# Alxaline/BraTS21

Measured on AMD Instinct MI355X. Metric: train patches/sec (4x128^3, width-48), higher is better.
Workload: dtype bf16; 1 GPU; equiunet width=48, batch=2/GPU of 4x128^3 synthetic patches, fwd + deep-supervision Dice + bwd + ranger (BASELINE.json configs[1]); global_batch=2, parallelism=dp1

## Files before the change

### brats21_amd/csrc/conv_wgrad.hip

```cpp
#include <stdlib.h>
#include "twin_begin.hpp"
#include "common.hpp"

typedef __attribute__((ext_vector_type(4))) short s16x4;

struct WgradParams {
  const void* x1; const void* x2; int c1, c2, p1, p2;
  const void* dy; int dyp;
  float* ws;
  int N, D, H, W, cin, cout;
  int tz, ty, tx, ntiles, nsplit;
  int nlane;
  int ntaps, dil;
  int seglen, nsegz;
};

constexpr int WG_TZ = 4, WG_TY = 4, WG_TX = 16, WG_VOX = 256;

template <typename T, int DIL, int COF, int CIF, int KS = 3>
struct WgGeom {
  static constexpr bool BF = std::is_same<T, bf16_t>::value;
  static constexpr int ESZ = sizeof(T);
  static constexpr int EPL = 16 / ESZ;
  static constexpr int R = KS == 3 ? DIL : 0;
// ... 543 lines not shown
      const int yoff = ybase + (32 * s) * G::SY;
#pragma unroll
      for (int m = 0; m < COF; ++m) a[s & 1][m] = tr_pair(ldy + yoff + m * 32, ldy + yoff + 16 * G::SY + m * 32);
    };
    auto read_b = [&](auto u_) {
      constexpr int u = u_;
      constexpr int s = u / G::PPW, jj = u % G::PPW;
      const int xoff = xbase + (((s >> 1) * G::HY + 2 * (s & 1)) * G::HX) * G::SX + poff[jj];
      b[u % (PD + 1)] = tr_pair(ldx + xoff, ldx + xoff + G::HX * G::SX);
    };
    constexpr int NU = 8 * G::PPW;
    static_for<0, G::XI>([&](auto i_) { issue_x(L, i_); });
    static_for<0, G::YI>([&](auto i_) { issue_y(L, i_); });
    __builtin_amdgcn_sched_barrier(0);
    read_a(std::integral_constant<int, 0>{});
    static_for<0, PD>([&](auto u_) { read_b(u_); });
    static_for<0, NU>([&](auto u_) {
      constexpr int u = u_;
      constexpr int s = u / G::PPW, jj = u % G::PPW;
      if constexpr (u + PD < NU) read_b(std::integral_constant<int, u + PD>{});
      if constexpr (jj == 0 && s + 1 < 8) read_a(std::integral_constant<int, s + 1>{});
      __builtin_amdgcn_sched_barrier(0);
#pragma unroll
      for (int m = 0; m < COF; ++m)
        acc[jj][m] = MFMA16_16x16x32(a[s & 1][m], b[u % (PD + 1)], acc[jj][m]);
      __builtin_amdgcn_sched_barrier(0);
    });
  }

#ifdef BRATS_WGRAD_STAMPS
  WG_STAMP(4);
  if (lane == 0 && blockIdx.y == 0 && blockIdx.z == 0) {
    long long* st = (long long*)(p.ws + (size_t)gridDim.x * 27 * p.cout * p.cin) + ((size_t)blockIdx.x * 8 + wave) * 5;
    for (int i = 0; i < 5; ++i) st[i] = tacc[i];
  }
#endif
#pragma unroll
  for (int jj = 0; jj < G::PPW; ++jj) {
    const int pid = wave + 8 * jj;
    if (pid < G::PAIRS) {
      const int t = pid / CIF, nn = pid % CIF;
      float* base = p.ws + ((size_t)split * 27 + t) * p.cout * p.cin;
      const int ci = ci0 + nn * 16 + v;
      if (CIF > 1 || ci < p.cin) {
#pragma unroll
        for (int m = 0; m < COF; ++m)
#pragma unroll
          for (int r = 0; r < 4; ++r) base[(size_t)(co0 + m * 16 + 4 * q + r) * p.cin + ci] = acc[jj][m][r];
      }
    }
  }
}

template <int COF, int CIF> struct Wg3f {
  static constexpr int HZ = WG_TZ + 2, HY = WG_TY + 2, HX = WG_TX + 2, HVOX = HZ * HY * HX;
  static constexpr int CO = 16 * COF, CI = 16 * CIF;
  static constexpr int SX = CI, SY = CO;
  static constexpr int XPPV = CI / 8, YPPV = CO / 8;
  static constexpr int XPIECES = HVOX * XPPV, YPIECES = WG_VOX * YPPV;
  static constexpr int XI = (XPIECES + 511) / 512, YI = YPIECES / 512;
  static constexpr int XB = XI * 512 * 16, YB = YI * 512 * 16;
  static constexpr int LDS_X = HVOX * SX;
  static constexpr int LDS = XB + YB + LDS_X + WG_VOX * SY;
  static constexpr int PAIRS = 27 * CIF, PPW = (PAIRS + 7) / 8;
  static_assert(YPIECES % 512 == 0, "");
};

template <int STRIDE> DEVI i32x8 tr8_frag(const char* base, int o0, int o1) {
  typedef __attribute__((ext_vector_type(2))) int v2i;
  typedef __attribute__((address_space(3))) v2i* lp;
  const v2i a0 = __builtin_amdgcn_ds_read_tr8_b64_v2i32((lp)(base + o0));
  const v2i a1 = __builtin_amdgcn_ds_read_tr8_b64_v2i32((lp)(base + o0 + 8 * STRIDE));
  const v2i a2 = __builtin_amdgcn_ds_read_tr8_b64_v2i32((lp)(base + o1));
  const v2i a3 = __builtin_amdgcn_ds_read_tr8_b64_v2i32((lp)(base + o1 + 8 * STRIDE));
  return i32x8{a0[0], a0[1], a1[0], a1[1], a2[0], a2[1], a3[0], a3[1]};
}

struct WgradF8Params { WgradParams w; const float* amax_x1; const float* amax_x2; const float* amax_dy; };

template <int COF, int CIF>
__global__ __launch_bounds__(512, 1) void conv_wgrad_alltaps_f8_kernel(const WgradF8Params pp) {
  typedef bf16_t T;
  using G = Wg3f<COF, CIF>;
  const WgradParams& p = pp.w;
  extern __shared__ __attribute__((aligned(16))) char lds[];
  char* ldx = lds + G::XB + G::YB;
  char* ldy = ldx + G::LDS_X;
  const int tid = threadIdx.x, lane = tid & 63;
  const int wave = __builtin_amdgcn_readfirstlane(tid >> 6);
  const int kq = lane >> 4, L = lane & 15;
  const int lane8 = blockIdx.x % p.nlane, gsub = blockIdx.x / p.nlane, g8 = gridDim.x / p.nlane;
  const int split = blockIdx.x;
  const int tpx = (p.ntiles + p.nlane - 1) / p.nlane;
  const int tile_end = min(p.ntiles, (lane8 + 1) * tpx);
  const int co0 = blockIdx.y * G::CO, ci0 = blockIdx.z * G::CI;
  const T* xsrc;
  int xpitch;
  if (ci0 < p.c1) { xsrc = (const T*)p.x1 + ci0; xpitch = p.p1; }
  else { xsrc = (const T*)p.x2 + (ci0 - p.c1); xpitch = p.p2; }
  const int xpb = xpitch * 2, ypb = p.dyp * 2;
  float ax = *pp.amax_x1;
  if (pp.amax_x2) ax = fmaxf(ax, *pp.amax_x2);
  const float xs = f8_scale_from_amax(ax), ys = f8_scale_from_amax(*pp.amax_dy);

  int xoffs[G::XI], xcode[G::XI];
#pragma unroll
// ... 273 lines not shown
  return t;
}
static WgradParams wgrad_params(const WgradArgs& a, float* ws, const WgradTileGrid& t, int nlane, int nsplit, int ntaps, int dil) {
  WgradParams p{};
  p.x1 = a.x1; p.x2 = a.x2; p.c1 = a.c1; p.c2 = a.c2; p.p1 = a.p1; p.p2 = a.p2;
  p.dy = a.dy; p.dyp = a.dyp; p.ws = ws;
  p.N = a.N; p.D = a.D; p.H = a.H; p.W = a.W; p.cin = a.cin(); p.cout = a.cout;
  p.tz = t.tz; p.ty = t.ty; p.tx = t.tx; p.ntiles = t.ntiles;
  p.nlane = nlane; p.nsplit = nsplit; p.ntaps = ntaps; p.dil = dil;
  return p;
}

static int wgrad_nlane(int ntiles) {
  int nl = 8;
  while (nl > 1 && ntiles / nl < 16) nl >>= 1;
  return nl;
}
static int wgrad_split_g8(int ntiles, int nlane, int groups, int cot, int cit) {
  int g8 = ceil_div(512, groups * nlane * cot * cit);
  const int cap = ceil_div(ntiles, nlane);
  if (g8 > cap) g8 = cap;
  return g8 < 1 ? 1 : g8;
}
static bool wgrad_blocks_g8(int ntiles, int blocks, int* nlane, int* g8) {
  *nlane = wgrad_nlane(ntiles);
  *g8 = ceil_div(device_cus(), *nlane * blocks);
  if (*g8 < 1) *g8 = 1;
  return ntiles >= 4 * *nlane * *g8;
}
static void wgrad_tiles(int dtype, int c1, int c2, int cout, int* cof, int* cif) {
  const int co16 = ceil_div(cout, 16);
  *cof = co16 % 3 == 0 ? 3 : (co16 % 2 == 0 ? 2 : 1);
  if (dtype == BRATS_F32) { *cif = 1; return; }
  const int a = ceil_div(c1, 16), b = c2 > 0 ? ceil_div(c2, 16) : 0;
  auto ok = [&](int f) { return a % f == 0 && (b == 0 || b % f == 0); };
  *cif = ok(3) ? 3 : (ok(2) ? 2 : 1);
}

int g_wgrad_alltaps_mode = -1;
extern "C" int BRATS_API(brats_conv3d_set_wgrad_alltaps)(int mode) {
  const int old = g_wgrad_alltaps_mode;
  g_wgrad_alltaps_mode = mode < 0 ? -1 : (mode ? 1 : 0);
  return old;
}
static int wgrad_alltaps_mode() {
  static int env_mode = -1;
  if (env_mode < 0) {
    const char* e = getenv("BRATS_WGRAD_ALLTAPS");
    env_mode = e ? atoi(e) : 1;
  }
  return g_wgrad_alltaps_mode >= 0 ? g_wgrad_alltaps_mode : env_mode;
}

enum WgradForm {
  WG_TAP_PLANE, WG_SHIFTED_TAP,
  WG_ALLTAPS2_33, WG_ALLTAPS2_42, WG_ALLTAPS2_31,
  WG_ALLTAPS_1, WG_ALLTAPS_1_4,
  WG_F8_33, WG_F8_42
};
struct WgradPlan {
  WgradForm form;
  int cof, cif;
  int cot, cit;
  int nlane, g8, nsplit;
  int ntaps, groups;
  bool clear;
  WgradTileGrid tiles;
  size_t per;
  size_t slab_bytes() const { return nsplit * per * sizeof(float); }
};

static WgradPlan wgrad_plan(int dtype, bool shifted, int ksize, int dil, const WgradArgs& a) {
  WgradPlan pl;
  const int c1 = a.c1, c2 = a.c2, cin = a.cin(), cout = a.cout;
  pl.tiles = wgrad_tile_grid(a);
  pl.ntaps = ksize == 3 ? 27 : 1;
  pl.per = (size_t)pl.ntaps * cout * cin;
  const bool narrow = c2 == 0 && c1 <= 16;
  auto blocks_of = [&](int co, int ci) { return cout % co == 0 && (narrow || (c1 % ci == 0 && c2 % ci == 0)); };
  if (!shifted && wgrad_alltaps_mode() && dtype == BRATS_BF16 && dil == 1 && (blocks_of(48, 48) || blocks_of(64, 32))) {
    const bool wide = !blocks_of(48, 48);
    pl.cof = wide ? 4 : 3; pl.cif = narrow ? 1 : (wide ? 2 : 3);
    pl.cot = cout / (16 * pl.cof); pl.cit = narrow ? 1 : cin / (16 * pl.cif);
    if (wgrad_blocks_g8(pl.tiles.ntiles, pl.cot * pl.cit, &pl.nlane, &pl.g8)) {
      pl.form = wide ? (narrow ? WG_ALLTAPS_1_4 : WG_ALLTAPS2_42) : narrow ? (c1 % 8 == 0 ? WG_ALLTAPS2_31 : WG_ALLTAPS_1) : WG_ALLTAPS2_33;
      pl.groups = 1;
      pl.clear = false;
      pl.nsplit = pl.nlane * pl.g8;
      return pl;
    }
  }
  pl.form = shifted ? WG_SHIFTED_TAP : WG_TAP_PLANE;
  wgrad_tiles(dtype, c1, c2, cout, &pl.cof, &pl.cif);
  pl.cot = ceil_div(cout, 16 * pl.cof);
  pl.cit = ceil_div(c1, 16 * pl.cif) + (c2 > 0 ? ceil_div(c2, 16 * pl.cif) : 0);
  pl.groups = shifted ? pl.ntaps : 3;
  pl.nlane = wgrad_nlane(pl.tiles.ntiles);
  pl.g8 = wgrad_split_g8(pl.tiles.ntiles, pl.nlane, pl.groups, pl.cot, pl.cit);
  pl.nsplit = pl.nlane * pl.g8;
  pl.clear = cin % 16 || cout % 16;
  return pl;
}
static size_t wgrad_slab_room(int dtype, bool shifted, int ksize, const WgradArgs& a) {
  const size_t d1 = wgrad_plan(dtype, shifted, ksize, 1, a).slab_bytes();
  const size_t d2 = shifted ? 0 : wgrad_plan(dtype, shifted, ksize, 2, a).slab_bytes();
  return d1 > d2 ? d1 : d2;
}

template <typename T, int DIL, int COF, int CIF, int KS = 3>
static int wgrad_launch(const WgradParams& p, dim3 grid, hipStream_t st) {
  using G = WgGeom<T, DIL, COF, CIF, KS>;
  auto kern = conv_wgrad_kernel<T, DIL, COF, CIF, KS>;
  static std::atomic<uint64_t> attr_done{0};
  BRATS_ENSURE_LDS_ATTR(kern, G::LDS, attr_done);
  hipLaunchKernelGGL(kern, grid, dim3(256), G::LDS, st, p);
  BRATS_CHECK_LAUNCH();
  return 0;
}

template <typename T, int DIL, int KS = 3>
static int wgrad_dispatch(const WgradParams& p, int cof, int cif, dim3 grid, hipStream_t st) {
#define WG_CASE(A, B) if (cof == A && cif == B) return wgrad_launch<T, DIL, A, B, KS>(p, grid, st);
  WG_CASE(3, 1) WG_CASE(2, 1) WG_CASE(1, 1)
  if constexpr (std::is_same<T, bf16_t>::value) {
    WG_CASE(3, 3) WG_CASE(3, 2) WG_CASE(2, 3) WG_CASE(2, 2) WG_CASE(1, 3) WG_CASE(1, 2)
  }
#undef WG_CASE
  BRATS_FAIL(BRATS_E_UNSUPPORTED, "wgrad: unsupported tile %dx%d", cof, cif);
}

template <auto KERN, int LDS>
static int wgrad_alltaps_launch(const WgradParams& p, dim3 grid, hipStream_t st) {
  static std::atomic<uint64_t> attr_done{0};
  BRATS_ENSURE_LDS_ATTR(KERN, LDS, attr_done);
  hipLaunchKernelGGL(KERN, grid, dim3(512), LDS, st, p);
  BRATS_CHECK_LAUNCH();
  return 0;
}

static int wgrad_run(const WgradPlan& pl, int dtype, int dil, const WgradArgs& a, float* ws, size_t room, hipStream_t st) {
  const char* who = pl.form == WG_SHIFTED_TAP ? "wgrad_shift" : "wgrad";
  if (a.c2 > 0 && a.c1 % (16 * pl.cif)) BRATS_FAIL(BRATS_E_UNSUPPORTED, "wgrad: c1=%d must be a multiple of the ci tile %d", a.c1, 16 * pl.cif);
  if (pl.slab_bytes() > room) BRATS_FAIL(BRATS_E_ARG, "%s: the plan's %zu bytes of slabs exceed the workspace size %zu", who, pl.slab_bytes(), room);
  const WgradParams p = wgrad_params(a, ws, pl.tiles, pl.nlane, pl.nsplit, pl.ntaps, dil);
  if (pl.clear) {
    hipError_t e = hipMemsetAsync(ws, 0, pl.slab_bytes(), st);
    if (e != hipSuccess) BRATS_FAIL(BRATS_E_HIP, "%s: memset: %s", who, hipGetErrorString(e));
  }
  const dim3 grid(pl.groups * pl.nsplit, pl.cot, pl.cit);
  const bool bf = dtype == BRATS_BF16;
  switch (pl.form) {
    case WG_TAP_PLANE:
      if (bf) return dil == 1 ? wgrad_dispatch<bf16_t, 1>(p, pl.cof, pl.cif, grid, st) : wgrad_dispatch<bf16_t, 2>(p, pl.cof, pl.cif, grid, st);
      return dil == 1 ? wgrad_dispatch<float, 1>(p, pl.cof, pl.cif, grid, st) : wgrad_dispatch<float, 2>(p, pl.cof, pl.cif, grid, st);
    case WG_SHIFTED_TAP:
      return bf ? wgrad_dispatch<bf16_t, 1, 1>(p, pl.cof, pl.cif, grid, st) : wgrad_dispatch<float, 1, 1>(p, pl.cof, pl.cif, grid, st);
    case WG_ALLTAPS2_33: return wgrad_alltaps_launch<conv_wgrad_alltaps2_kernel<3, 3>, Wg3b<3, 3>::LDS>(p, grid, st);
    case WG_ALLTAPS2_42: return wgrad_alltaps_launch<conv_wgrad_alltaps2_kernel<4, 2>, Wg3b<4, 2>::LDS>(p, grid, st);
    case WG_ALLTAPS2_31: return wgrad_alltaps_launch<conv_wgrad_alltaps2_kernel<3, 1>, Wg3b<3, 1>::LDS>(p, grid, st);
    case WG_ALLTAPS_1: return wgrad_alltaps_launch<conv_wgrad_alltaps_kernel<1>, Wg3<1>::LDS>(p, grid, st);
    case WG_ALLTAPS_1_4: return wgrad_alltaps_launch<conv_wgrad_alltaps_kernel<1, 4>, Wg3<1, 4>::LDS>(p, grid, st);
    default: BRATS_FAIL(BRATS_E_UNSUPPORTED, "wgrad: form %d is not a 16-bit / f32 kernel", (int)pl.form);
  }
}

template <int V>
__global__ void __launch_bounds__(256) x3_split_kernel(const float* __restrict__ src, int pitch, bf16_t* __restrict__ hi,
                                                       bf16_t* __restrict__ lo, size_t voxels, int C, const float* __restrict__ amax) {
  const float sc = amax ? x3_scale_from_amax(*amax) : 1.f;
  const int cv = C / 8;
  const size_t total = voxels * cv;
  const size_t stride = (size_t)gridDim.x * 256;
  auto load = [&](size_t i, u32x4& a, u32x4& b) {
    const float* p = src + (i / cv) * pitch + (i % cv) * 8;
    a = __builtin_nontemporal_load((const u32x4*)p);
    b = __builtin_nontemporal_load((const u32x4*)(p + 4));
  };
  auto emit = [&](size_t i, const u32x4& a, const u32x4& b) {
    const uint32_t w[8] = {a[0], a[1], a[2], a[3], b[0], b[1], b[2], b[3]};
    uint32_t h[4], l[4];
#pragma unroll
    for (int e = 0; e < 4; ++e) {
      const float x0 = __uint_as_float(w[2 * e]) * sc, x1 = __uint_as_float(w[2 * e + 1]) * sc;
      x3_split2(x0, x1, h[e], l[e]);
    }
    const size_t o = (i / cv) * C + (i % cv) * 8;
    __builtin_nontemporal_store(u32x4{h[0], h[1], h[2], h[3]}, (u32x4*)(hi + o));
    __builtin_nontemporal_store(u32x4{l[0], l[1], l[2], l[3]}, (u32x4*)(lo + o));
  };
  size_t i = (size_t)blockIdx.x * 256 + threadIdx.x;
  for (; i + stride < total; i += 2 * stride) {
    u32x4 a0, b0, a1, b1;
    load(i, a0, b0);
    load(i + stride, a1, b1);
    emit(i, a0, b0);
    emit(i + stride, a1, b1);
  }
  if (i < total) {
    u32x4 a0, b0;
    load(i, a0, b0);
    emit(i, a0, b0);
  }
}
static size_t x3_align(size_t b) { return (b + 255) / 256 * 256; }
// ... 9 lines not shown
  X3Carve(size_t room16, const WgradArgs& a) {
    const int c[3] = {a.c1, a.c2, a.cout};
    size_t b = x3_align(3 * room16);
    for (int i = 0; i < 6; ++i) {
      off[i] = b;
      b += c[i / 2] > 0 ? x3_align(a.vox() * c[i / 2] * 2) : 0;
    }
    off[6] = b;
  }
  size_t bytes() const { return off[6]; }
  bf16_t* at(float* ws, int i) const { return (bf16_t*)((char*)ws + off[i]); }
};

static int wgrad_x3(const WgradPlan& pl, int dil, const WgradArgs& a, const float* amax_dy, float* ws, float* dw, size_t room16,
                          hipStream_t st) {
  const X3Carve cv(room16, a);
  bf16_t *h1 = cv.at(ws, 0), *l1 = cv.at(ws, 1), *h2 = cv.at(ws, 2), *l2 = cv.at(ws, 3), *hy = cv.at(ws, 4), *ly = cv.at(ws, 5);
  x3_split_launch((const float*)a.x1, a.p1, h1, l1, a.vox(), a.c1, nullptr, st);
  if (a.c2 > 0) x3_split_launch((const float*)a.x2, a.p2, h2, l2, a.vox(), a.c2, nullptr, st);
  x3_split_launch((const float*)a.dy, a.dyp, hy, ly, a.vox(), a.cout, amax_dy, st);
  BRATS_CHECK_LAUNCH();
  WgradArgs t = a;
  t.p1 = a.c1; t.p2 = a.c2; t.dyp = a.cout;
  const bool xlo[3] = {true, false, false}, ylo[3] = {false, true, false};
  for (int k = 0; k < 3; ++k) {
    t.x1 = xlo[k] ? l1 : h1;
    t.x2 = a.c2 > 0 ? (xlo[k] ? l2 : h2) : nullptr;
    t.dy = ylo[k] ? ly : hy;
    const int rc = wgrad_run(pl, BRATS_BF16, dil, t, ws + (size_t)k * pl.nsplit * pl.per, room16, st);
    if (rc) return rc;
  }
  wgrad_reduce_launch((const float*)ws, dw, 3 * pl.nsplit, a.cout, a.cin(), pl.ntaps, st, amax_dy);
  return 0;
}

#include "conv_wgrad_x3.hpp"
extern "C" int BRATS_API(brats_conv3d_set_x3_wgrad_fused)(int mode) {
  const int old = g_x3_wgrad_fused_mode;
  g_x3_wgrad_fused_mode = mode < 0 ? -1 : (mode > 2 ? 2 : mode);
  return old;
}

static size_t wgrad_ws_bytes(int dtype, bool shifted, int ksize, const WgradArgs& a) {
  if (dtype != BRATS_X3_BF16) return wgrad_slab_room(dtype, shifted, ksize, a);
  const size_t three = X3Carve(wgrad_slab_room(BRATS_BF16, shifted, ksize, a), a).bytes();
  const size_t fused = shifted ? 0 : wgrad_x3_fused_ws_bytes(a);
  return three > fused ? three : fused;
}
extern "C" size_t BRATS_API(brats_conv3d_wgrad_ws_bytes)(int dtype, int ksize, int N, int D, int H, int W, int c1, int c2, int cout) {
  return ksize == 3 ? wgrad_ws_bytes(dtype, false, 3, wgrad_shape(N, D, H, W, c1, c2, cout)) : 0;
}
extern "C" size_t BRATS_API(brats_conv3d_wgrad_shift_ws_bytes)(int dtype, int ksize, int N, int D, int H, int W, int cin, int cout) {
  return ksize == 1 || ksize == 3 ? wgrad_ws_bytes(dtype, true, ksize, wgrad_shape(N, D, H, W, cin, 0, cout)) : 0;
}

static int wgrad_impl(bool shifted, WgradArgs a, const float* amax_dy, float* ws, float* dw, float* dbias, int dtype, int ksize, int dil,
                      brats_stream_t s) {
  const char* who = shifted ? "wgrad_shift" : "wgrad";
  if (!a.x1 || !a.dy || !ws || !dw || a.c1 <= 0 || a.cout <= 0 || (shifted && (a.N <= 0 || a.D <= 0 || a.H <= 0 || a.W <= 0)))
    BRATS_FAIL(BRATS_E_ARG, "%s: null pointer / bad size", who);
  if (shifted ? (ksize != 1 && ksize != 3) || dil < 1 : ksize != 3 || (dil != 1 && dil != 2))
    BRATS_FAIL(BRATS_E_UNSUPPORTED, "%s: ksize=%d dil=%d unsupported", who, ksize, dil);
  if (shifted && dtype != BRATS_BF16 && dtype != BRATS_F32 && dtype != BRATS_X3_BF16) BRATS_FAIL(BRATS_E_UNSUPPORTED, "wgrad_shift: dtype %d", dtype);
  if (a.c2 < 0) a.c2 = 0;
  if (a.c2 > 0 && !a.x2) BRATS_FAIL(BRATS_E_ARG, "wgrad: c2 > 0 but x2 NULL");
  const bool x3 = dtype == BRATS_X3_BF16;
  const int epl = vec_width(dtype);
  if (a.p1 % epl || (a.c2 && a.p2 % epl) || a.dyp % epl || a.c1 % epl || a.c2 % epl || a.cout % epl)
    BRATS_FAIL(BRATS_E_ARG, "%s: channel counts / pitches must be multiples of %d", who, epl);
  if (x3 && (a.c1 % 8 || a.c2 % 8 || a.cout % 8)) BRATS_FAIL(BRATS_E_ARG, "%s (split precision): channel counts must be multiples of 8", who);
  if (const int mp = wgrad_sample_overflow(a, dtype == BRATS_BF16 ? 2 : 4))
    BRATS_FAIL(BRATS_E_UNSUPPORTED, "%s: one sample of %dx%dx%d x pitch %d exceeds the 2 GiB buffer-offset range", who, a.D, a.H, a.W, mp);
  hipStream_t st = (hipStream_t)s;
  int rc = x3 && !shifted ? wgrad_x3_fused(a, amax_dy, ws, dw, dil, st) : 1;
  if (rc == 1) {
    const int dt = x3 ? BRATS_BF16 : dtype;
    const WgradPlan pl = wgrad_plan(dt, shifted, ksize, dil, a);
    const size_t room = wgrad_slab_room(dt, shifted, ksize, a);
    if (x3) rc = wgrad_x3(pl, dil, a, amax_dy, ws, dw, room, st);
    else if (!(rc = wgrad_run(pl, dtype, dil, a, ws, room, st))) wgrad_reduce_launch((const float*)ws, dw, pl.nsplit, a.cout, a.cin(), pl.ntaps, st);
  }
  if (rc) return rc;
  if (dbias) wgrad_dbias_launch(dtype, a.dy, a.dyp, dbias, a.vox(), a.cout, st);
  BRATS_CHECK_LAUNCH();
  return 0;
}

extern "C" int BRATS_API(brats_conv3d_wgrad)(const void* x1, int c1, int pitch1, const void* x2, int c2, int pitch2, const void* dy,
                                  int dypitch, float* ws, float* dw, float* dbias, int dtype, int ksize, int dil, int N,
                                  int D, int H, int W, int cout, brats_stream_t s) {
  return wgrad_impl(false, WgradArgs{x1, c1, pitch1, x2, c2, pitch2, dy, dypitch, N, D, H, W, cout}, nullptr, ws, dw, dbias, dtype, ksize, dil, s);
}
extern "C" int BRATS_API(brats_conv3d_x3_wgrad)(const void* x1, int c1, int pitch1, const void* x2, int c2, int pitch2, const void* dy,
                                     int dypitch, const float* amax_dy, float* ws, float* dw, float* dbias, int dtype, int dil,
                                     int N, int D, int H, int W, int cout, brats_stream_t s) {
  if (dtype != BRATS_X3_BF16) BRATS_FAIL(BRATS_E_ARG, "conv3d_x3_wgrad: dtype must be BRATS_X3_F16 or BRATS_X3_BF16");
  return wgrad_impl(false, WgradArgs{x1, c1, pitch1, x2, c2, pitch2, dy, dypitch, N, D, H, W, cout}, amax_dy, ws, dw, dbias, dtype, 3, dil, s);
}
extern "C" int BRATS_API(brats_conv3d_wgrad_shift)(const void* x, int cin, int xpitch, const void* dy, int dypitch, float* ws, float* dw,
                                        float* dbias, int dtype, int ksize, int dil, int N, int D, int H, int W, int cout,
                                        brats_stream_t s) {
  return wgrad_impl(true, WgradArgs{x, cin, xpitch, nullptr, 0, 0, dy, dypitch, N, D, H, W, cout}, nullptr, ws, dw, dbias, dtype, ksize, dil, s);
}
extern "C" int BRATS_API(brats_conv3d_x3_wgrad_shift)(const void* x, int cin, int xpitch, const void* dy, int dypitch, const float* amax_dy,
                                           float* ws, float* dw, float* dbias, int dtype, int ksize, int dil, int N, int D, int H,
                                           int W, int cout, brats_stream_t s) {
  if (dtype != BRATS_X3_BF16) BRATS_FAIL(BRATS_E_ARG, "conv3d_x3_wgrad_shift: dtype must be BRATS_X3_F16 or BRATS_X3_BF16");
  return wgrad_impl(true, WgradArgs{x, cin, xpitch, nullptr, 0, 0, dy, dypitch, N, D, H, W, cout}, amax_dy, ws, dw, dbias, dtype, ksize, dil, s);
}

static bool wgrad_f8_plan(const WgradArgs& a, WgradPlan* pl) {
  const int c1 = a.c1, c2 = a.c2, cout = a.cout;
  if (c1 <= 0 || cout <= 0) return false;
  if (cout % 48 == 0 && c1 % 48 == 0 && c2 % 48 == 0) { pl->form = WG_F8_33; pl->cof = 3; pl->cif = 3; }
  else if (cout % 64 == 0 && c1 % 32 == 0 && c2 % 32 == 0) { pl->form = WG_F8_42; pl->cof = 4; pl->cif = 2; }
  else return false;
  pl->tiles = wgrad_tile_grid(a);
  pl->cot = cout / (16 * pl->cof); pl->cit = a.cin() / (16 * pl->cif);
  if (!wgrad_blocks_g8(pl->tiles.ntiles, pl->cot * pl->cit, &pl->nlane, &pl->g8)) return false;
  pl->nsplit = pl->nlane * pl->g8;
  pl->ntaps = 27; pl->groups = 1; pl->clear = false;
  pl->per = (size_t)27 * cout * a.cin();
  return true;
}

extern "C" size_t BRATS_API(brats_conv3d_wgrad_f8_ws_bytes)(int N, int D, int H, int W, int c1, int c2, int cout) {
  WgradPlan pl;
  return wgrad_f8_plan(wgrad_shape(N, D, H, W, c1, c2, cout), &pl) ? pl.slab_bytes() : 0;
}

template <int COF, int CIF>
static int wgrad_f8_launch(const WgradF8Params& pp, dim3 grid, hipStream_t st) {
// ... 33 lines not shown
```

### brats21_amd/csrc/gen_twin_dispatch.py

```python
#!/usr/bin/env python3
import re
import sys

BOTH = {"brats_conv3d_set_vs8", "brats_conv3d_set_kp", "brats_conv3d_set_wgrad_alltaps", "brats_conv3d_set_x3_wgrad_fused",
        "brats_upsample_bwd_set_fused"}
DATA = {"brats_conv3d_f8_fwd", "brats_conv3d_wgrad_f8", "brats_conv3d_pack_weights_multi"}

txt = re.sub(r"/\*.*?\*/", " ", open(sys.argv[1]).read(), flags=re.S)
protos = {}
for m in re.finditer(r"(const char\s*\*|size_t|int)\s+(brats_[a-z0-9_]+)\s*\(([^)]*)\)\s*;", txt):
    protos[m.group(2)] = (" ".join(m.group(1).split()), " ".join(m.group(3).split()))
names = []
for path in sys.argv[2:]:
    for m in re.finditer(r'extern "C" [a-z_ \*]+?BRATS_API\((brats_[a-z0-9_]+)\)\(', open(path).read()):
        names.append(m.group(1))
print("// GENERATED by gen_twin_dispatch.py from include/brats_hip.h -- do not edit")
print('#include "../../include/brats_hip.h"')
print('extern "C" {')
for n in names:
    if n not in protos:
        raise SystemExit(f"{n} is defined in a twinned translation unit but not declared in brats_hip.h")
    ret, args = protos[n]
    arglist = [] if args in ("", "void") else [a.strip() for a in args.split(",")]
    argnames = [re.search(r"([A-Za-z_][A-Za-z0-9_]*)$", a).group(1) for a in arglist]
    call = ", ".join(argnames)
    sig = args if arglist else "void"
    print(f"{ret} {n}_bf16({sig});")
    print(f"{ret} {n}_f16({sig});")
    if n in DATA:
        if n + "_f16" not in protos:
            raise SystemExit(f"{n}_f16 must be declared in brats_hip.h (16-bit data, no dtype argument)")
        print(f"{ret} {n}({sig}) {{ return {n}_bf16({call}); }}")
    elif n in BOTH:
        print(f"{ret} {n}({sig}) {{ {n}_f16({call}); return {n}_bf16({call}); }}")
    elif "dtype" in argnames:
        call16 = ", ".join("BRATS_BF16" if a == "dtype" else a for a in argnames)
        callx3 = ", ".join("BRATS_X3_BF16" if a == "dtype" else a for a in argnames)
        print(f"{ret} {n}({sig}) {{ return dtype == BRATS_F16 ? {n}_f16({call16}) : dtype == BRATS_X3_F16 ? {n}_f16({callx3}) : {n}_bf16({call}); }}")
    else:
        print(f"{ret} {n}({sig}) {{ return {n}_bf16({call}); }}")
print("}")
```

### include/brats_hip.h

```cpp
#ifndef BRATS_HIP_H
#define BRATS_HIP_H
#include <stddef.h>
#include <stdint.h>

#ifdef __cplusplus
extern "C" {
#endif

typedef void* brats_stream_t;

enum { BRATS_F32 = 0, BRATS_BF16 = 1, BRATS_F16 = 2, BRATS_X3_BF16 = 3, BRATS_X3_F16 = 4 };
enum { BRATS_E_ARG = -1, BRATS_E_UNSUPPORTED = -2, BRATS_E_HIP = -3 };
enum { BRATS_ACT_NONE = 0, BRATS_ACT_RELU = 1, BRATS_ACT_LEAKY = 2, BRATS_ACT_ELU = 3, BRATS_ACT_SWISH = 4, BRATS_ACT_MISH = 5 };

#define BRATS_ABI_VERSION 7
int brats_abi_version(void);
const char* brats_last_error(void);

int brats_dropout(const void* x, int xpitch, void* out, int opitch, int dtype, size_t voxels, int C, float p,
                  const void* state, int unit, brats_stream_t s);

int brats_ncdhw_to_ndhwc(const float* src, void* dst, int dtype, int N, int C, int cpad, int dst_pitch,
                         int D, int H, int W, brats_stream_t s);
int brats_ndhwc_to_ncdhw(const void* src, int src_pitch, float* dst, int dtype, int N, int C,
// ... 3 lines not shown
size_t brats_conv3d_packed_bytes(int dtype, int ksize, int cin, int cout, int ck);
int brats_conv3d_chunk(int dtype, int ksize, int dil, int c1, int c2, int cout);
int brats_conv3d_pack_weights(const float* w, void* packed, int dtype, int mode, int ksize,
                              int cout_w, int cin_w, int cin_off, int cin_cnt, int ck, brats_stream_t s);
typedef struct {
  const float* w;
  void* out;
  int dtype, mode, taps, cin_w, cin_real, cin_off, rows, rows16, kdim, ck, ms_n, reserved;
  unsigned long long total;
} brats_pack_job;
int brats_conv3d_pack_blocks(int kdim, int ck, int rows);
int brats_conv3d_pack_weights_multi(const brats_pack_job* jobs, const int* blocks , int nblocks,
                                    brats_stream_t s);
int brats_conv3d_pack_weights_multi_f16(const brats_pack_job* jobs, const int* blocks , int nblocks,
                                    brats_stream_t s);
int brats_conv3d_tiles_per_sample(int D, int H, int W);
int brats_conv3d_split_granule(int cout);
int brats_conv3d_set_vs8(int mode);
int brats_conv3d_set_kp(int mode);
int brats_conv3d_fwd(const void* x1, int c1, int pitch1, const void* x2, int c2, int pitch2,
                     const void* packed_w, const float* bias, void* y, int ypitch,
                     void* y2, int y2pitch, int ysplit, float* stats,
                     int dtype, int ksize, int dil, int N, int D, int H, int W, int cout,
                     brats_stream_t s);
int brats_conv3d_pre_ok(int dtype, int ksize, int dil, int c1, int c2, int cout);
int brats_conv3d_fwd_pre(const void* x1, int c1, int pitch1, const float* ss1, const void* x2, int c2, int pitch2,
                         const float* ss2, int act, float slope, const void* packed_w, const float* bias, void* y, int ypitch,
                         float* stats, int dtype, int dil, int N, int D, int H, int W, int cout, brats_stream_t s);
int brats_conv3d_bstats_ok(int dtype, int ksize, int dil, int c1, int cout);
int brats_conv3d_fwd_bstats(const void* x1, int c1, int pitch1, const void* packed_w, void* y, int ypitch,
                            const void* fwd_y, int fwd_pitch, const float* scale_shift, int act, float slope,
                            float* tile_stats, int dtype, int dil, int N, int D, int H, int W, int cout, brats_stream_t s);
int brats_conv3d_x3_fwd(const void* x1, int c1, int pitch1, const void* x2, int c2, int pitch2, const float* xamax,
                        const void* packed_w, const float* bias, void* y, int ypitch, void* y2, int y2pitch, int ysplit,
                        float* stats, int dtype, int dil, int N, int D, int H, int W, int cout, brats_stream_t s);
int brats_conv3d_x3_fwd_bstats(const void* x1, int c1, int pitch1, const float* xamax, const void* packed_w, void* y, int ypitch,
                               const void* fwd_y, int fwd_pitch, const float* scale_shift, int act, float slope,
                               float* tile_stats, int dtype, int dil, int N, int D, int H, int W, int cout, brats_stream_t s);
int brats_conv3d_f8_chunk(int c1, int c2);
size_t brats_conv3d_f8_packed_bytes(int cin, int cout, int ck);
int brats_conv3d_f8_pack_weights(const float* w, void* packed, int mode, int cout_w, int cin_w, int cin_off,
                                 int cin_cnt, int ck, brats_stream_t s);
int brats_conv3d_f8_fwd(const void* x1, int c1, int pitch1, const float* amax1, const void* x2, int c2, int pitch2,
                        const float* amax2, float xscale, const void* packed_w, const float* bias, void* y, int ypitch,
                        void* y2, int y2pitch, int ysplit, float* stats, int dil, int N, int D, int H, int W, int cout,
                        brats_stream_t s);
int brats_conv3d_f8_fwd_f16(const void* x1, int c1, int pitch1, const float* amax1, const void* x2, int c2, int pitch2,
                        const float* amax2, float xscale, const void* packed_w, const float* bias, void* y, int ypitch,
                        void* y2, int y2pitch, int ysplit, float* stats, int dil, int N, int D, int H, int W, int cout,
                        brats_stream_t s);
int brats_absmax(const void* x, int pitch, int dtype, size_t rows, int C, float* out, brats_stream_t s);
size_t brats_conv3d_wgrad_ws_bytes(int dtype, int ksize, int N, int D, int H, int W, int c1, int c2, int cout);
int brats_conv3d_set_wgrad_alltaps(int mode);
int brats_conv3d_set_x3_wgrad_fused(int mode);
int brats_conv3d_wgrad(const void* x1, int c1, int pitch1, const void* x2, int c2, int pitch2,
                       const void* dy, int dypitch, float* ws, float* dw, float* dbias,
                       int dtype, int ksize, int dil, int N, int D, int H, int W, int cout,
                       brats_stream_t s);
int brats_conv3d_x3_wgrad(const void* x1, int c1, int pitch1, const void* x2, int c2, int pitch2, const void* dy, int dypitch,
                          const float* amax_dy, float* ws, float* dw, float* dbias, int dtype, int dil, int N, int D, int H,
                          int W, int cout, brats_stream_t s);
size_t brats_conv3d_wgrad_f8_ws_bytes(int N, int D, int H, int W, int c1, int c2, int cout);
int brats_conv3d_wgrad_f8(const void* x1, int c1, int pitch1, const float* amax1, const void* x2, int c2, int pitch2,
                          const float* amax2, const void* dy, int dypitch, const float* amax_dy, float* ws, float* dw,
                          int N, int D, int H, int W, int cout, brats_stream_t s);
int brats_conv3d_wgrad_f8_f16(const void* x1, int c1, int pitch1, const float* amax1, const void* x2, int c2, int pitch2,
                          const float* amax2, const void* dy, int dypitch, const float* amax_dy, float* ws, float* dw,
                          int N, int D, int H, int W, int cout, brats_stream_t s);
size_t brats_conv3d_wgrad_shift_ws_bytes(int dtype, int ksize, int N, int D, int H, int W, int cin, int cout);
int brats_conv3d_wgrad_shift(const void* x, int cin, int xpitch, const void* dy, int dypitch, float* ws, float* dw,
                             float* dbias, int dtype, int ksize, int dil, int N, int D, int H, int W, int cout,
                             brats_stream_t s);
int brats_conv3d_x3_wgrad_shift(const void* x, int cin, int xpitch, const void* dy, int dypitch, const float* amax_dy,
                                float* ws, float* dw, float* dbias, int dtype, int ksize, int dil, int N, int D, int H, int W,
                                int cout, brats_stream_t s);

size_t brats_gn_ws_doubles(int N, int C);
int brats_gn_finalize(const float* stats, int tiles_per_sample, int N, int C, int groups,
                      double count_per_channel, float eps, const float* gamma, const float* beta,
                      float* mean_rstd , float* scale_shift ,
                      double* chan_ws , brats_stream_t s);
int brats_affine_act_fwd(const void* y, int ypitch, const float* scale_shift, void* z, int zpitch,
                         int dtype, int act, float slope, const float* slope_dev, int N, int voxels, int C, float* amax,
                         brats_stream_t s);
int brats_affine_act_pool_fwd(const void* y, int ypitch, const float* scale_shift, void* z, int zpitch, void* pooled,
                              int ppitch, unsigned char* argmax ,
                              int dtype, int act, float slope, const float* slope_dev, int N, int D, int H, int W, int C,
                              int with_avg, float* amax, brats_stream_t s);
size_t brats_gn_bwd_ws_floats(int N, int C);
int brats_gn_act_bwd(const void* dz, int dzpitch, const void* y, int ypitch, const float* scale_shift,
                     const float* mean_rstd, const float* gamma, void* dy, int dypitch,
                     float* red , float* dgamma, float* dbeta,
                     int dtype, int act, float slope, const float* slope_dev, int N, int voxels, int C, int groups,
                     float* amax , brats_stream_t s);
int brats_gn_act_bwd_tiles(const float* tile_stats, int tiles_per_sample, const void* dz, int dzpitch, const void* y,
                           int ypitch, const float* scale_shift, const float* mean_rstd, const float* gamma, void* dy,
                           int dypitch, float* red , float* dgamma, float* dbeta, int dtype, int act,
                           float slope, int N, int voxels, int C, int groups,
                           float* amax , brats_stream_t s);
size_t brats_gn_bwd_head_ws_floats(int N, int C, int K);
int brats_gn_act_bwd_head(const float* dlogits, const float* hw, int K, const void* y, int ypitch, const float* scale_shift,
                          const float* mean_rstd, const float* gamma, void* dy, int dypitch, float* red ,
                          float* hws, float* dgamma, float* dbeta, float* dhw, float* dhb, int dtype, int act, float slope,
                          int N, int voxels, int C, int groups, float* amax, brats_stream_t s);
int brats_gn_act_bwd_pool(const void* dskip, int dskip_pitch, const void* dpool, int dpool_pitch, const unsigned char* argmax,
                          const void* y, int ypitch, const float* scale_shift, const float* mean_rstd, const float* gamma,
// ... 306 lines not shown
```

Baseline: 138.7 patches/s.

## Add warp-specialized no-slab wgrad kernel for small-spatial bf16 convolutions

Adds a bf16 weight-gradient kernel for 3x3x3 convolutions. Each workgroup owns one 48x16 cout/cin block and walks every spatial tile itself, writing dw directly instead of per-split slabs that a separate reduction then sums. Four loader waves double-buffer halo and dy tiles into LDS via async DMA while eight MFMA waves accumulate all 27 taps, and results are transposed through LDS for coalesced stores. By default it is chosen only when the channel grid fills most CUs and the spatial tile count is small (deep, low-resolution layers), trading less split parallelism for no slab traffic and no reduction launch.

```diff
diff --git a/brats21_amd/csrc/conv_wgrad.hip b/brats21_amd/csrc/conv_wgrad.hip
--- a/brats21_amd/csrc/conv_wgrad.hip
+++ b/brats21_amd/csrc/conv_wgrad.hip
@@ -619,6 +619,218 @@
   }
 }
 
+template <int DIL> struct Wg3n {
+  static constexpr int HZ = WG_TZ + 2 * DIL, HY = WG_TY + 2 * DIL, HX = WG_TX + 2 * DIL, HVOX = HZ * HY * HX;
+  static constexpr int COF = 3, CO = 48, CI = 16;
+  static constexpr int SX = 2 * CI, SY = 2 * CO, XPPV = CI / 8, YPPV = CO / 8;
+  static constexpr int MMA_WAVES = 8, LOAD_WAVES = 4, THREADS = 64 * (MMA_WAVES + LOAD_WAVES), LT = 64 * LOAD_WAVES;
+  static constexpr int XPIECES = HVOX * XPPV, YPIECES = WG_VOX * YPPV;
+  static constexpr int XI = (XPIECES + LT - 1) / LT, YI = YPIECES / LT;
+  static constexpr int XB = XI * LT * 16, YB = YI * LT * 16;
+  static constexpr int BUF = XB + YB;
+  static constexpr int PAIRS = 27, PPW = 4;
+  static constexpr int OUT_ROW = CI * 27, OUT_B = CO * OUT_ROW * 4;
+  static constexpr int LDS = 2 * BUF > OUT_B ? 2 * BUF : OUT_B;
+  static_assert(HZ <= 8 && HY <= 8 && HX <= 32, "packed halo coordinates: 3 + 3 + 5 bits");
+  static_assert(YPIECES % LT == 0, "");
+};
+
+struct WgNoslabWalk {
+  int nlane, nsplit, g8, tpx, ntiles;
+  int split, tile, end;
+  DEVI void enter() {
+    for (;; ++split) {
+      const int lane8 = split % nlane;
+      tile = lane8 * tpx + split / nlane;
+      end = min(ntiles, (lane8 + 1) * tpx);
+      if (tile < end || split + 1 >= nsplit) return;
+    }
+  }
+  DEVI WgNoslabWalk(const WgradParams& p) : nlane(p.nlane), nsplit(p.nsplit), g8(p.nsplit / p.nlane),
+                                            tpx((p.ntiles + p.nlane - 1) / p.nlane), ntiles(p.ntiles), split(0) { enter(); }
+  DEVI bool done() const { return tile >= end; }
+  DEVI bool next() {
+    tile += g8;
+    if (tile < end) return false;
+    if (split + 1 < nsplit) { ++split; enter(); }
+    return true;
+  }
+};
+
+template <int DIL>
+__global__ __launch_bounds__(768, 1) void conv_wgrad_noslab_kernel(const WgradParams p) {
+  typedef bf16_t T;
+  using G = Wg3n<DIL>;
+  extern __shared__ __attribute__((aligned(16))) char lds[];
+  const int tid = threadIdx.x, lane = tid & 63;
+  const int wave = __builtin_amdgcn_readfirstlane(tid >> 6);
+  const int co0 = blockIdx.y * G::CO, ci0 = blockIdx.z * G::CI;
+  f32x4 tot[G::PPW][G::COF];
+#pragma unroll
+  for (int jj = 0; jj < G::PPW; ++jj)
+#pragma unroll
+    for (int m = 0; m < G::COF; ++m) tot[jj][m] = f32x4{0.f, 0.f, 0.f, 0.f};
+
+  WgNoslabWalk walk(p);
+  if (wave >= G::MMA_WAVES) {
+    const int lt = tid - 64 * G::MMA_WAVES, lw = wave - G::MMA_WAVES;
+    const T* xsrc;
+    int xpitch;
+    if (ci0 < p.c1) { xsrc = (const T*)p.x1 + ci0; xpitch = p.p1; }
+    else { xsrc = (const T*)p.x2 + (ci0 - p.c1); xpitch = p.p2; }
+    const int xpb = xpitch * 2, ypb = p.dyp * 2;
+    int xoffs[G::XI], xcode[G::XI], yoffs[G::YI], ycode[G::YI];
+#pragma unroll
+    for (int i = 0; i < G::XI; ++i) {
+      const int P = lt + G::LT * i;
+      const int vox = P / G::XPPV, part = P % G::XPPV;
+      const int hx = vox % G::HX, hy = (vox / G::HX) % G::HY, hz = vox / (G::HX * G::HY);
+      const bool ok = P < G::XPIECES;
+      xoffs[i] = ok ? ((hz * p.H + hy) * p.W + hx) * xpb + part * 16 : (int)0x80000000;
+      xcode[i] = ok ? (hz | hy << 3 | hx << 6 | 1 << 14) : 0;
+    }
+#pragma unroll
+    for (int i = 0; i < G::YI; ++i) {
+      const int P = lt + G::LT * i;
+      const int vox = P / G::YPPV, part = P % G::YPPV;
+      const int z = vox >> 6, y = (vox >> 4) & 3, x = vox & 15;
+      yoffs[i] = ((z * p.H + y) * p.W + x) * ypb + part * 16;
+      ycode[i] = (z + DIL) | (y + DIL) << 3 | (x + DIL) << 6;
+    }
+    const unsigned xsample_bytes = (unsigned)p.D * p.H * p.W * xpitch * 2;
+    const unsigned ysample_bytes = (unsigned)p.D * p.H * p.W * p.dyp * 2;
+    auto issue_tile = [&](int tile, int buf) {
+      int bt = tile;
+      const int x0 = (bt % p.tx) * WG_TX; bt /= p.tx;
+      const int y0 = (bt % p.ty) * WG_TY; bt /= p.ty;
+      const int z0 = (bt % p.tz) * WG_TZ;
+      const int n = bt / p.tz;
+      const size_t sample_vox = (size_t)n * p.D * p.H * p.W;
+      const rsrc4_t xrs = make_rsrc4(xsrc + sample_vox * xpitch, xsample_bytes);
+      const rsrc4_t yrs = make_rsrc4((const T*)p.dy + sample_vox * p.dyp + co0, ysample_bytes);
+      const int xorg = (((z0 - DIL) * p.H + (y0 - DIL)) * p.W + (x0 - DIL)) * xpb;
+      const int yorg = ((z0 * p.H + y0) * p.W + x0) * ypb;
+      char* const dst = lds + buf * G::BUF + lw * 1024;
+      auto inside = [](int o, int size, int hn) {
+        const int lo = o >= DIL ? 0 : DIL - o, hi = size - o + DIL < hn ? size - o + DIL : hn;
+        return hi > lo ? ((1u << hi) - 1u) & ~((1u << lo) - 1u) : 0u;
+      };
+      const unsigned zm = inside(z0, p.D, G::HZ), ym = inside(y0, p.H, G::HY), xm = inside(x0, p.W, G::HX);
+      static_for<0, G::XI>([&](auto i_) {
+        constexpr int i = i_;
+        const int c = xcode[i];
+        const unsigned ok = (unsigned)(c >> 14) & (zm >> (c & 7)) & (ym >> ((c >> 3) & 7)) & (xm >> ((c >> 6) & 31)) & 1u;
+        lds_dma16_async(xrs, dst + i * (G::LT * 16), (xorg + xoffs[i]) | ((int)ok - 1));
+      });
+      static_for<0, G::YI>([&](auto i_) {
+        constexpr int i = i_;
+        const int c = ycode[i];
+        const unsigned ok = (zm >> (c & 7)) & (ym >> ((c >> 3) & 7)) & (xm >> ((c >> 6) & 31)) & 1u;
+        lds_dma16_async(yrs, dst + G::XB + i * (G::LT * 16), (yorg + yoffs[i]) | ((int)ok - 1));
+      });
+    };
+    issue_tile(walk.tile, 0);
+    asm volatile("s_waitcnt vmcnt(0)" ::: "memory");
+    __syncthreads();
+    for (int buf = 1; !walk.done(); buf ^= 1) {
+      walk.next();
+      if (!walk.done()) issue_tile(walk.tile, buf);
+      asm volatile("s_waitcnt vmcnt(0)" ::: "memory");
+      __syncthreads();
+    }
+  } else {
+    const int q = lane >> 4, v = lane & 15;
+    const bool four = wave + 24 < G::PAIRS;
+    int poff[G::PPW];
+#pragma unroll
+    for (int jj = 0; jj < G::PPW; ++jj) {
+      const int t = wave + 8 * jj;
+      poff[jj] = t < G::PAIRS ? ((((t / 9) * G::HY + (t / 3) % 3) * G::HX + t % 3) * DIL) * G::SX : 0;
+    }
+    f32x4 acc[G::PPW][G::COF];
+#pragma unroll
+    for (int jj = 0; jj < G::PPW; ++jj)
+#pragma unroll
+      for (int m = 0; m < G::COF; ++m) acc[jj][m] = f32x4{0.f, 0.f, 0.f, 0.f};
+    const int qq = v >> 2, pp = v & 3;
+    const int ybase = (4 * q + qq) * G::SY + pp * 8;
+    const int xbase = (4 * q + qq) * G::SX + pp * 8;
+    __syncthreads();
+    for (int buf = 0; !walk.done(); buf ^= 1) {
+      const char* ldx = lds + buf * G::BUF;
+      const char* ldy = ldx + G::XB;
+      constexpr int PD = 3;
+      bf16x8 a[2][G::COF], b[PD + 1];
+      auto read_a = [&](auto s_) {
+        constexpr int s = s_;
+        const int yoff = ybase + (32 * s) * G::SY;
+#pragma unroll
+        for (int m = 0; m < G::COF; ++m) a[s & 1][m] = tr_pair(ldy + yoff + m * 32, ldy + yoff + 16 * G::SY + m * 32);
+      };
+      auto read_b = [&](auto u_) {
+        constexpr int u = u_;
+        constexpr int s = u / G::PPW, jj = u % G::PPW;
+        if (jj + 1 < G::PPW || four) {
+          const int xoff = xbase + (((s >> 1) * G::HY + 2 * (s & 1)) * G::HX) * G::SX + poff[jj];
+          b[u % (PD + 1)] = tr_pair(ldx + xoff, ldx + xoff + G::HX * G::SX);
+        }
+      };
+      constexpr int NU = 8 * G::PPW;
+      read_a(std::integral_constant<int, 0>{});
+      static_for<0, PD>([&](auto u_) { read_b(u_); });
+      static_for<0, NU>([&](auto u_) {
+        constexpr int u = u_;
+        constexpr int s = u / G::PPW, jj = u % G::PPW;
+        if constexpr (u + PD < NU) read_b(std::integral_constant<int, u + PD>{});
+        if constexpr (jj == 0 && s + 1 < 8) read_a(std::integral_constant<int, s + 1>{});
+        __builtin_amdgcn_sched_barrier(0);
+        if (jj + 1 < G::PPW || four) {
+#pragma unroll
+          for (int m = 0; m < G::COF; ++m)
+            acc[jj][m] = MFMA16_16x16x32(a[s & 1][m], b[u % (PD + 1)], acc[jj][m]);
+        }
+        __builtin_amdgcn_sched_barrier(0);
+      });
+      if (walk.next()) {
+#pragma unroll
+        for (int jj = 0; jj < G::PPW; ++jj)
+#pragma unroll
+          for (int m = 0; m < G::COF; ++m) { tot[jj][m] += acc[jj][m]; acc[jj][m] = f32x4{0.f, 0.f, 0.f, 0.f}; }
+      }
+      __syncthreads();
+    }
+  }
+
+  float* outl = (float*)lds;
+  if (wave < G::MMA_WAVES) {
+    const int q = lane >> 4, v = lane & 15;
+#pragma unroll
+    for (int jj = 0; jj < G::PPW; ++jj) {
+      const int t = wave + 8 * jj;
+      if (t < G::PAIRS) {
+#pragma unroll
+        for (int m = 0; m < G::COF; ++m)
+#pragma unroll
+          for (int r = 0; r < 4; ++r) outl[(m * 16 + 4 * q + r) * G::OUT_ROW + v * 27 + t] = tot[jj][m][r];
+      }
+    }
+  }
+  __syncthreads();
+  const size_t row_pitch = (size_t)p.cin * 27;
+  float* dst = p.ws + (size_t)co0 * row_pitch + (size_t)ci0 * 27;
+  if (((size_t)p.ws & 15) == 0) {
+    for (int i = tid; i < G::CO * (G::OUT_ROW / 4); i += G::THREADS) {
+      const int row = i / (G::OUT_ROW / 4), c = i % (G::OUT_ROW / 4);
+      *(f32x4*)(dst + row * row_pitch + c * 4) = *(const f32x4*)(outl + row * G::OUT_ROW + c * 4);
+    }
+  } else {
+    for (int i = tid; i < G::CO * G::OUT_ROW; i += G::THREADS) {
+      const int row = i / G::OUT_ROW, c = i % G::OUT_ROW;
+      dst[row * row_pitch + c] = outl[i];
+    }
+  }
+}
+
 template <int COF, int CIF> struct Wg3f {
   static constexpr int HZ = WG_TZ + 2, HY = WG_TY + 2, HX = WG_TX + 2, HVOX = HZ * HY * HX;
   static constexpr int CO = 16 * COF, CI = 16 * CIF;
@@ -998,9 +1210,34 @@
   return g_wgrad_alltaps_mode >= 0 ? g_wgrad_alltaps_mode : env_mode;
 }
 
+int g_wgrad_noslab_mode = -1;
+extern "C" int BRATS_API(brats_conv3d_set_wgrad_noslab)(int mode) {
+  const int old = g_wgrad_noslab_mode;
+  g_wgrad_noslab_mode = mode < 0 ? -1 : (mode ? 1 : 0);
+  return old;
+}
+static int wgrad_noslab_mode() {
+  static int env_mode = -2;
+  if (env_mode < -1) {
+    const char* e = getenv("BRATS_WGRAD_NOSLAB");
+    const int m = e ? atoi(e) : -1;
+    env_mode = m < 0 ? -1 : (m ? 1 : 0);
+  }
+  return g_wgrad_noslab_mode >= 0 ? g_wgrad_noslab_mode : env_mode;
+}
+static bool wgrad_noslab_built(int dtype, bool shifted, int ksize, int dil, const WgradArgs& a) {
+  return !shifted && ksize == 3 && dtype == BRATS_BF16 && (dil == 1 || dil == 2) && a.cout > 0 && a.cout % 48 == 0 && a.c1 > 0 &&
+         a.c1 % 16 == 0 && a.c2 % 16 == 0 && a.N > 0 && a.D > 0 && a.H > 0 && a.W > 0;
+}
+static bool wgrad_noslab_rule(const WgradArgs& a, int dil, int ntiles) {
+  const int wgs = (a.cout / 48) * (a.cin() / 16);
+  return 4 * wgs >= 3 * device_cus() && ntiles <= (dil == 2 ? 64 : 32);
+}
+
 enum WgradForm {
   WG_TAP_PLANE, WG_SHIFTED_TAP,
   WG_ALLTAPS2_33, WG_ALLTAPS2_42, WG_ALLTAPS2_31,
+  WG_NOSLAB,
   WG_ALLTAPS_1, WG_ALLTAPS_1_4,
   WG_F8_33, WG_F8_42
 };
@@ -1016,12 +1253,22 @@
   size_t slab_bytes() const { return nsplit * per * sizeof(float); }
 };
 
-static WgradPlan wgrad_plan(int dtype, bool shifted, int ksize, int dil, const WgradArgs& a) {
+static WgradPlan wgrad_plan(int dtype, bool shifted, int ksize, int dil, const WgradArgs& a, bool noslab = false) {
   WgradPlan pl;
   const int c1 = a.c1, c2 = a.c2, cin = a.cin(), cout = a.cout;
   pl.tiles = wgrad_tile_grid(a);
   pl.ntaps = ksize == 3 ? 27 : 1;
   pl.per = (size_t)pl.ntaps * cout * cin;
+  if (noslab && wgrad_alltaps_mode() && wgrad_noslab_mode() != 0 && wgrad_noslab_built(dtype, shifted, ksize, dil, a) &&
+      (wgrad_noslab_mode() == 1 || wgrad_noslab_rule(a, dil, pl.tiles.ntiles))) {
+    pl.form = WG_NOSLAB;
+    pl.cof = 3; pl.cif = 1;
+    pl.cot = cout / 48; pl.cit = cin / 16;
+    const WgradPlan slab = wgrad_plan(dtype, shifted, ksize, dil, a);
+    pl.nlane = slab.nlane; pl.g8 = slab.g8; pl.nsplit = 0; pl.groups = 1;
+    pl.clear = false;
+    return pl;
+  }
   const bool narrow = c2 == 0 && c1 <= 16;
   auto blocks_of = [&](int co, int ci) { return cout % co == 0 && (narrow || (c1 % ci == 0 && c2 % ci == 0)); };
   if (!shifted && wgrad_alltaps_mode() && dtype == BRATS_BF16 && dil == 1 && (blocks_of(48, 48) || blocks_of(64, 32))) {
@@ -1075,11 +1322,11 @@
   BRATS_FAIL(BRATS_E_UNSUPPORTED, "wgrad: unsupported tile %dx%d", cof, cif);
 }
 
-template <auto KERN, int LDS>
+template <auto KERN, int LDS, int THREADS = 512>
 static int wgrad_alltaps_launch(const WgradParams& p, dim3 grid, hipStream_t st) {
   static std::atomic<uint64_t> attr_done{0};
   BRATS_ENSURE_LDS_ATTR(KERN, LDS, attr_done);
-  hipLaunchKernelGGL(KERN, grid, dim3(512), LDS, st, p);
+  hipLaunchKernelGGL(KERN, grid, dim3(THREADS), LDS, st, p);
   BRATS_CHECK_LAUNCH();
   return 0;
 }
@@ -1096,6 +1343,13 @@
   const dim3 grid(pl.groups * pl.nsplit, pl.cot, pl.cit);
   const bool bf = dtype == BRATS_BF16;
   switch (pl.form) {
+    case WG_NOSLAB: {
+      const dim3 g1(1, pl.cot, pl.cit);
+      WgradParams pn = p;
+      pn.nsplit = pl.nlane * pl.g8;
+      return dil == 1 ? wgrad_alltaps_launch<conv_wgrad_noslab_kernel<1>, Wg3n<1>::LDS, Wg3n<1>::THREADS>(pn, g1, st)
+                      : wgrad_alltaps_launch<conv_wgrad_noslab_kernel<2>, Wg3n<2>::LDS, Wg3n<2>::THREADS>(pn, g1, st);
+    }
     case WG_TAP_PLANE:
       if (bf) return dil == 1 ? wgrad_dispatch<bf16_t, 1>(p, pl.cof, pl.cif, grid, st) : wgrad_dispatch<bf16_t, 2>(p, pl.cof, pl.cif, grid, st);
       return dil == 1 ? wgrad_dispatch<float, 1>(p, pl.cof, pl.cif, grid, st) : wgrad_dispatch<float, 2>(p, pl.cof, pl.cif, grid, st);
@@ -1211,6 +1465,11 @@
 }
 extern "C" size_t BRATS_API(brats_conv3d_wgrad_shift_ws_bytes)(int dtype, int ksize, int N, int D, int H, int W, int cin, int cout) {
   return ksize == 1 || ksize == 3 ? wgrad_ws_bytes(dtype, true, ksize, wgrad_shape(N, D, H, W, cin, 0, cout)) : 0;
+}
+
+extern "C" int BRATS_API(brats_conv3d_wgrad_noslab_taken)(int dtype, int dil, int N, int D, int H, int W, int c1, int c2, int cout) {
+  if (dtype != BRATS_BF16 || c1 <= 0 || cout <= 0 || N <= 0 || D <= 0 || H <= 0 || W <= 0) return 0;
+  return wgrad_plan(dtype, false, 3, dil, wgrad_shape(N, D, H, W, c1, c2, cout), true).form == WG_NOSLAB ? 1 : 0;
 }
 
 static int wgrad_impl(bool shifted, WgradArgs a, const float* amax_dy, float* ws, float* dw, float* dbias, int dtype, int ksize, int dil,
@@ -1234,9 +1493,10 @@
   int rc = x3 && !shifted ? wgrad_x3_fused(a, amax_dy, ws, dw, dil, st) : 1;
   if (rc == 1) {
     const int dt = x3 ? BRATS_BF16 : dtype;
-    const WgradPlan pl = wgrad_plan(dt, shifted, ksize, dil, a);
+    const WgradPlan pl = wgrad_plan(dt, shifted, ksize, dil, a, !x3);
     const size_t room = wgrad_slab_room(dt, shifted, ksize, a);
     if (x3) rc = wgrad_x3(pl, dil, a, amax_dy, ws, dw, room, st);
+    else if (pl.form == WG_NOSLAB) rc = wgrad_run(pl, dtype, dil, a, dw, room, st);
     else if (!(rc = wgrad_run(pl, dtype, dil, a, ws, room, st))) wgrad_reduce_launch((const float*)ws, dw, pl.nsplit, a.cout, a.cin(), pl.ntaps, st);
   }
   if (rc) return rc;
diff --git a/brats21_amd/csrc/gen_twin_dispatch.py b/brats21_amd/csrc/gen_twin_dispatch.py
--- a/brats21_amd/csrc/gen_twin_dispatch.py
+++ b/brats21_amd/csrc/gen_twin_dispatch.py
@@ -2,8 +2,8 @@
 import re
 import sys
 
-BOTH = {"brats_conv3d_set_vs8", "brats_conv3d_set_kp", "brats_conv3d_set_wgrad_alltaps", "brats_conv3d_set_x3_wgrad_fused",
-        "brats_upsample_bwd_set_fused"}
+BOTH = {"brats_conv3d_set_vs8", "brats_conv3d_set_kp", "brats_conv3d_set_wgrad_alltaps", "brats_conv3d_set_wgrad_noslab",
+        "brats_conv3d_set_x3_wgrad_fused", "brats_upsample_bwd_set_fused"}
 DATA = {"brats_conv3d_f8_fwd", "brats_conv3d_wgrad_f8", "brats_conv3d_pack_weights_multi"}
 
 txt = re.sub(r"/\*.*?\*/", " ", open(sys.argv[1]).read(), flags=re.S)
diff --git a/include/brats_hip.h b/include/brats_hip.h
--- a/include/brats_hip.h
+++ b/include/brats_hip.h
@@ -79,6 +79,8 @@
 int brats_absmax(const void* x, int pitch, int dtype, size_t rows, int C, float* out, brats_stream_t s);
 size_t brats_conv3d_wgrad_ws_bytes(int dtype, int ksize, int N, int D, int H, int W, int c1, int c2, int cout);
 int brats_conv3d_set_wgrad_alltaps(int mode);
+int brats_conv3d_set_wgrad_noslab(int mode);
+int brats_conv3d_wgrad_noslab_taken(int dtype, int dil, int N, int D, int H, int W, int c1, int c2, int cout);
 int brats_conv3d_set_x3_wgrad_fused(int mode);
 int brats_conv3d_wgrad(const void* x1, int c1, int pitch1, const void* x2, int c2, int pitch2,
                        const void* dy, int dypitch, float* ws, float* dw, float* dbias,
```

After: 140.2 patches/s, median of 6. +1.1%, better.
